# ov2slam/ov2slam

Measured on AMD Instinct MI355X. Metric: frames/sec tracking + local-BA iters/sec, EuRoC MH_01 stereo 'accurate', 1 GPU vs CPU ref, higher is better.
Workload: dtype u8/int32 fixed point + f32 (LK), f64 (BA)

## Files before the change

### ov2slam_amd/csrc/clahe.hip

```cpp
#include "common.hpp"
#include "xcd_map.hpp"
#include <math.h>
#include <mutex>
#include <type_traits>

#pragma clang fp contract(off)

__device__ __forceinline__ int c_reflect101(int p, int len)
{
    if (len == 1) return 0;
    while (p < 0 || p >= len) p = p < 0 ? -p : 2 * len - 2 - p;
    return p;
}

struct ClaheParams {
    int w, h, stride, tiles_x, tiles_y, tw, th, clip;
    float lut_scale, inv_tw, inv_th;
    long long src_item_stride, dst_item_stride;
    int dst_stride;
    int border;
    int batch, gx_lut;
    int ysplit;
    int nstrips, nlut;
    long long l1_delta;
    int l1_pitch, l1_w, l1_h;
};

__device__ __forceinline__ void clahe_wave_sync()
{
    __builtin_amdgcn_fence(__ATOMIC_RELEASE, "wavefront");
    __builtin_amdgcn_wave_barrier();
    __builtin_amdgcn_fence(__ATOMIC_ACQUIRE, "wavefront");
}

#define CH_WAVE_DW 256
#define CH_CSTRIDE 264
#define CH_NCOPY 4
#define CH_MULTI_DW (CH_NCOPY * CH_CSTRIDE)
typedef uint32_t c_u32x4 __attribute__((ext_vector_type(4)));

template <int CTRL>
__device__ __forceinline__ int c_dpp0(int v) { return __builtin_amdgcn_update_dpp(0, v, CTRL, 0xF, 0xF, true); }

template <bool SRC_ALIGNED, class StoreLut>
__device__ __forceinline__ void clahe_lut_tiles(const ClaheParams &P, const uint8_t *img, uint32_t *hw, int lane, int t, int t_end, int tstride,
                                                StoreLut store_lut, int ncopy = 1)
{
    const int ntiles = t_end;
    const int sub = lane >> 4, l16 = lane & 15;
    uint32_t *hist = hw + ((lane ^ (lane >> 4)) & (ncopy - 1)) * CH_CSTRIDE;
    const bool fast_geom = P.tw <= 61 && P.th <= 64;
    const uint8_t *img_end = img + (long long)(P.h - 1) * P.stride + P.w;
    const bool same_phase = SRC_ALIGNED || (P.stride & 3) == 0;

    auto tile_fast = [&](int t) { const int xb = (t % P.tiles_x) * P.tw; return fast_geom && 2 * xb + P.tw <= 2 * P.w - 1; };
    const uint32_t lane_off = (uint32_t)(sub * P.stride + 4 * l16);
    auto tile_load = [&](int t, uint32_t (&vv)[16], uint32_t &phs) {
        const int ty = t / P.tiles_x, tx = t - ty * P.tiles_x;
        const int x_begin = tx * P.tw;
        if (SRC_ALIGNED && (ty * P.th + 64 <= P.h) && (long long)P.h * P.stride < (1ll << 31)) {
            const uint32_t ph = (uint32_t)(x_begin & 3);
            phs = ph * 0x55555555u;
            const uint8_t *tp = img + (long long)(ty * P.th) * P.stride + (x_begin & ~3);
            uint32_t off = (4 * l16 < P.tw + (int)ph && (x_begin & ~3) + 4 * l16 < P.w) ? lane_off : (uint32_t)(sub * P.stride);
#pragma unroll
            for (int i = 0; i < 16; i++) {
                vv[i] = *(const uint32_t *)(tp + off);
                off += 4u * (uint32_t)P.stride;
            }
            return;
        }
        const int ybase = ty * P.th + sub;
        phs = 0;
#pragma unroll
        for (int i = 0; i < 16; i++) {
            int y = ybase + 4 * i;
            y = y >= P.h ? 2 * P.h - 2 - y : y;
            y = y < 0 ? 0 : y;
            uint32_t v = 0;
            if (SRC_ALIGNED) {
                const uint32_t ph = (uint32_t)(x_begin & 3);
                phs |= ph << (2 * i);
                if (4 * i + sub < P.th && 4 * l16 < P.tw + (int)ph && (x_begin & ~3) + 4 * l16 < P.w) v = *(const uint32_t *)(img + y * P.stride + (x_begin & ~3) + 4 * l16);
            } else {
                const uint8_t *rp = img + (long long)y * P.stride + x_begin;
                const uint32_t ph = (uint32_t)((size_t)rp & 3);
                phs |= ph << (2 * i);
                const uint8_t *ap = rp - ph + 4 * l16;
                if (4 * i + sub < P.th && 4 * l16 < P.tw + (int)ph && x_begin - (int)ph + 4 * l16 < P.w) {
                    if (ap + 4 <= img_end) v = *(const uint32_t *)ap;
                    else for (int k = 0; k < 4; k++) if (ap + k < img_end) v |= (uint32_t)ap[k] << (8 * k);
                }
            }
            vv[i] = v;
        }
    };

    uint32_t cur[16], cur_ph = 0;
    auto histogram = [&](int th) {
        const int ty = th / P.tiles_x, tx = th - ty * P.tiles_x;
        const int x_begin = tx * P.tw;
        if (ncopy == 1) ((c_u32x4 *)hw)[lane] = (c_u32x4)(0u);
        else for (int q = lane; q < CH_MULTI_DW / 4; q += 64) ((c_u32x4 *)hw)[q] = (c_u32x4)(0u);
        clahe_wave_sync();
        if (tile_fast(th)) {
            const int dbl_lo = 2 * P.w - 2 - (x_begin + P.tw);
            auto wgt = [&](int p) { const int c = x_begin + p; return ((unsigned)p < (unsigned)P.tw && c < P.w) ? ((c > dbl_lo && c <= P.w - 2) ? 2u : 1u) : 0u; };
            const int p_same = 4 * l16 - (int)(cur_ph & 3);
            uint32_t w0 = wgt(p_same), w1 = wgt(p_same + 1), w2 = wgt(p_same + 2), w3 = wgt(p_same + 3);
            bool mine = p_same < P.tw;
#pragma unroll
            for (int i = 0; i < 16; i++) {
                if (!same_phase) {
                    const int p0 = 4 * l16 - (int)((cur_ph >> (2 * i)) & 3);
                    w0 = wgt(p0); w1 = wgt(p0 + 1); w2 = wgt(p0 + 2); w3 = wgt(p0 + 3);
                    mine = p0 < P.tw;
                }
                if (mine && 4 * i + sub < P.th) {
                    const uint32_t v = cur[i];
                    atomicAdd(&hist[v & 0xFF], w0);
                    atomicAdd(&hist[(v >> 8) & 0xFF], w1);
                    atomicAdd(&hist[(v >> 16) & 0xFF], w2);
                    atomicAdd(&hist[v >> 24], w3);
                }
            }
        } else {
            for (int ly = sub; ly < P.th; ly += 4) {
                const uint8_t *row = img + (long long)c_reflect101(ty * P.th + ly, P.h) * P.stride;
                for (int lx = l16; lx < P.tw; lx += 16) atomicAdd(&hist[row[c_reflect101(x_begin + lx, P.w)]], 1u);
            }
        }
    };
    if (t < ntiles) {
        if (tile_fast(t)) tile_load(t, cur, cur_ph);
        histogram(t);
        if (t + tstride < ntiles && tile_fast(t + tstride)) tile_load(t + tstride, cur, cur_ph);
    }
#pragma nounroll
    for (; t < ntiles; t += tstride) {
        clahe_wave_sync();
        int hv[4];
        {
            c_u32x4 q = *(const c_u32x4 *)(hw + 4 * lane);
            for (int c = 1; c < ncopy; c++) q += *(const c_u32x4 *)(hw + c * CH_CSTRIDE + 4 * lane);
            hv[0] = (int)q.x; hv[1] = (int)q.y; hv[2] = (int)q.z; hv[3] = (int)q.w;
        }
        clahe_wave_sync();
        const int tn = t + tstride;
        if (tn < ntiles) {
            histogram(tn);
            if (tn + tstride < ntiles && tile_fast(tn + tstride)) tile_load(tn + tstride, cur, cur_ph);
        }
        if (P.clip > 0) {
            int over = 0;
#pragma unroll
            for (int k = 0; k < 4; k++) { over += max(hv[k] - P.clip, 0); hv[k] = min(hv[k], P.clip); }
            over += c_dpp0<0xB1>(over); over += c_dpp0<0x4E>(over); over += c_dpp0<0x124>(over); over += c_dpp0<0x128>(over);
            const int clipped = __builtin_amdgcn_readlane(over, 0) + __builtin_amdgcn_readlane(over, 16) +
                                __builtin_amdgcn_readlane(over, 32) + __builtin_amdgcn_readlane(over, 48);
            const int batch = clipped >> 8, residual = clipped & 255;
            int step = residual ? (int)(256.0f / (float)residual) : 1;
            int q = (int)((float)(4 * lane) / (float)step), r = 4 * lane - q * step;
#pragma unroll
            for (int k = 0; k < 4; k++) {
                hv[k] += batch + ((residual != 0 && r == 0 && q < residual) ? 1 : 0);
                r++;
                if (r == step) { r = 0; q++; }
            }
        }
        hv[1] += hv[0]; hv[2] += hv[1]; hv[3] += hv[2];
        int v = hv[3];
        v += c_dpp0<0x111>(v); v += c_dpp0<0x112>(v); v += c_dpp0<0x114>(v); v += c_dpp0<0x118>(v);
        const int r0 = __builtin_amdgcn_readlane(v, 15), r1 = __builtin_amdgcn_readlane(v, 31), r2 = __builtin_amdgcn_readlane(v, 47);
        const int rowoff = sub == 0 ? 0 : (sub == 1 ? r0 : (sub == 2 ? r0 + r1 : r0 + r1 + r2));
        const int base = v + rowoff - hv[3];
        uint32_t packed = 0;
#pragma unroll
        for (int k = 0; k < 4; k++) {
            int r = __float2int_rn((float)(hv[k] + base) * P.lut_scale);
            r = r < 0 ? 0 : (r > 255 ? 255 : r);
            packed |= (uint32_t)r << (8 * k);
        }
        store_lut(t, packed);
    }
}

template <bool SRC_ALIGNED>
__global__ __launch_bounds__(256, 4) void k_clahe_lut(ClaheParams P, const uint8_t *__restrict__ src, uint8_t *__restrict__ lut)
{
    __shared__ __attribute__((aligned(16))) uint32_t hist_all[4][CH_MULTI_DW];
    const int wave = __builtin_amdgcn_readfirstlane(threadIdx.x >> 6), lane = threadIdx.x & 63;
    const int ntiles = P.tiles_x * P.tiles_y;
    int b, bx;
    ov2_xcd_map(blockIdx.x, P.gx_lut, P.batch, &b, &bx);
    uint8_t *lb = lut + (long long)b * ntiles * 256 + 4 * lane;
    clahe_lut_tiles<SRC_ALIGNED>(P, src + (long long)b * P.src_item_stride, hist_all[wave], lane, bx * 4 + wave, ntiles, 4 * P.gx_lut,
                                 [&](int t, uint32_t packed) { *(uint32_t *)(lb + (long long)t * 256) = packed; }, CH_NCOPY);
}

#define CLAHE_MAX_CELLS 48
#define CA_UNROLL 6
typedef float c_f32x2 __attribute__((ext_vector_type(2)));

__device__ __forceinline__ float c_ub(uint32_t q, int k) { return (float)((q >> (8 * k)) & 0xFFu); }

template <bool SRC_ALIGNED>
__global__ __launch_bounds__(512) void k_clahe_apply(ClaheParams P, const uint8_t *__restrict__ src, const uint8_t *__restrict__ lut,
                                                     uint8_t *__restrict__ dst)
{
    extern __shared__ __align__(16) unsigned char clahe_smem[];
    const int ncx = P.tiles_x + 1;
    uint32_t *lut4 = (uint32_t *)clahe_smem;
    int cy, b;
    ov2_xcd_map(blockIdx.x, (P.tiles_y + 1) * P.ysplit, P.batch, &b, &cy);
    const int part = cy % P.ysplit;
    cy /= P.ysplit;
    const int tid = threadIdx.x, nthr = blockDim.x;
    const int ty1 = max(cy - 1, 0), ty2 = min(cy, P.tiles_y - 1);
    const uint8_t *L = lut + (long long)b * P.tiles_x * P.tiles_y * 256;
    for (int e = tid; e < ncx * 64; e += nthr) {
        const int cx = e >> 6, v4 = (e & 63) * 4;
        const int tx1 = max(cx - 1, 0), tx2 = min(cx, P.tiles_x - 1);
        const uint32_t a = *(const uint32_t *)(L + (ty1 * P.tiles_x + tx1) * 256 + v4), bb = *(const uint32_t *)(L + (ty1 * P.tiles_x + tx2) * 256 + v4);
        const uint32_t c = *(const uint32_t *)(L + (ty2 * P.tiles_x + tx1) * 256 + v4), d = *(const uint32_t *)(L + (ty2 * P.tiles_x + tx2) * 256 + v4);
        const uint32_t ab01 = __builtin_amdgcn_perm(bb, a, 0x05010400u), ab23 = __builtin_amdgcn_perm(bb, a, 0x07030602u);
        const uint32_t cd01 = __builtin_amdgcn_perm(d, c, 0x05010400u), cd23 = __builtin_amdgcn_perm(d, c, 0x07030602u);
        c_u32x4 o;
        o.x = __builtin_amdgcn_perm(cd01, ab01, 0x05040100u); o.y = __builtin_amdgcn_perm(cd01, ab01, 0x07060302u);
        o.z = __builtin_amdgcn_perm(cd23, ab23, 0x05040100u); o.w = __builtin_amdgcn_perm(cd23, ab23, 0x07060302u);
        *(c_u32x4 *)(lut4 + (cx << 8) + v4) = o;
    }
    __syncthreads();
    int y0 = max(0, (int)floorf(((float)cy - 0.5f) * (float)P.th) - 1), y1 = min(P.h, (int)ceilf(((float)cy + 0.5f) * (float)P.th) + 2);
    while (y0 < y1 && (int)floorf((float)y0 * P.inv_th - 0.5f) + 1 != cy) y0++;
    while (y1 > y0 && (int)floorf((float)(y1 - 1) * P.inv_th - 0.5f) + 1 != cy) y1--;
    if (P.ysplit > 1) {
        const int chunk = (y1 - y0 + P.ysplit - 1) / P.ysplit;
        y0 = min(y1, y0 + part * chunk);
        y1 = min(y1, y0 + chunk);
    }
    const uint8_t *simg = src + (long long)b * P.src_item_stride;
    uint8_t *dimg = dst + (long long)b * P.dst_item_stride;
    const bool dst_aligned = ((P.dst_stride | (int)(size_t)dimg) & 3) == 0;
    constexpr bool src_aligned = SRC_ALIGNED;
    const uint8_t *simg_end = simg + (long long)(P.h - 1) * P.stride + P.w;
    const int ndw = (P.w + 3) >> 2;
    for (int dwi = tid; dwi < ndw; dwi += nthr) {
        const int xb = 4 * dwi;
        float xa[4], xa1[4];
        const uint32_t *lutc[4];
#pragma unroll
        for (int k = 0; k < 4; k++) {
            const int x = min(xb + k, P.w - 1);
            const float txf = (float)x * P.inv_tw - 0.5f;
            const int fx = (int)floorf(txf);
            xa[k] = txf - (float)fx; xa1[k] = 1.0f - xa[k];
            lutc[k] = lut4 + ((fx + 1) << 8);
        }
        const c_f32x2 XA01 = {xa[0], xa[1]}, XA23 = {xa[2], xa[3]}, XB01 = {xa1[0], xa1[1]}, XB23 = {xa1[2], xa1[3]};
        const bool full = dst_aligned && xb + 3 < P.w;
        auto load_rows = [&](int yb, uint32_t (&inr)[CA_UNROLL]) {
#pragma unroll
            for (int u = 0; u < CA_UNROLL; u++) {
                const int y = min(yb + u, y1 - 1);
                const uint8_t *sp = simg + (long long)y * P.stride + xb;
                uint32_t in = 0;
                if (src_aligned) in = *(const uint32_t *)sp;
                else {
                    const uint32_t ph = (uint32_t)((size_t)sp & 3);
                    const uint8_t *ap = sp - ph;
                    if (xb + 3 < P.w && ap + 8 <= simg_end) {
                        const uint32_t lo = *(const uint32_t *)ap, hi = *(const uint32_t *)(ap + 4);
                        in = __builtin_amdgcn_alignbyte(hi, lo, ph);
                    } else for (int k = 0; k < 4; k++) if (xb + k < P.w) in |= (uint32_t)sp[k] << (8 * k);
                }
                inr[u] = in;
            }
        };
        uint32_t inr[CA_UNROLL], nxt[CA_UNROLL];
        if (y0 < y1) load_rows(y0, inr);
        for (int yb = y0; yb < y1; yb += CA_UNROLL) {
            load_rows(yb + CA_UNROLL, nxt);
#pragma unroll
            for (int u = 0; u < CA_UNROLL; u++) {
                const int y = yb + u;
                if (y >= y1) break;
                const float tyf = (float)y * P.inv_th - 0.5f;
                const float ya = tyf - (float)(cy - 1), ya1 = 1.0f - ya;
                const c_f32x2 YA = {ya, ya}, YB = {ya1, ya1};
                uint8_t *drow = dimg + y * P.dst_stride;
                const uint32_t in = inr[u];
                const uint32_t q0 = lutc[0][in & 0xFF], q1 = lutc[1][(in >> 8) & 0xFF], q2 = lutc[2][(in >> 16) & 0xFF], q3 = lutc[3][in >> 24];
                const c_f32x2 A11 = {c_ub(q0, 0), c_ub(q1, 0)}, A12 = {c_ub(q0, 1), c_ub(q1, 1)}, A21 = {c_ub(q0, 2), c_ub(q1, 2)}, A22 = {c_ub(q0, 3), c_ub(q1, 3)};
                const c_f32x2 B11 = {c_ub(q2, 0), c_ub(q3, 0)}, B12 = {c_ub(q2, 1), c_ub(q3, 1)}, B21 = {c_ub(q2, 2), c_ub(q3, 2)}, B22 = {c_ub(q2, 3), c_ub(q3, 3)};
                const c_f32x2 r01 = (A11 * XB01 + A12 * XA01) * YB + (A21 * XB01 + A22 * XA01) * YA;
                const c_f32x2 r23 = (B11 * XB23 + B12 * XA23) * YB + (B21 * XB23 + B22 * XA23) * YA;
                uint32_t out = __builtin_amdgcn_cvt_pk_u8_f32(rintf(r01.x), 0, 0u);
                out = __builtin_amdgcn_cvt_pk_u8_f32(rintf(r01.y), 1, out);
                out = __builtin_amdgcn_cvt_pk_u8_f32(rintf(r23.x), 2, out);
                out = __builtin_amdgcn_cvt_pk_u8_f32(rintf(r23.y), 3, out);
                if (full) *(uint32_t *)(drow + xb) = out;
                else for (int k = 0; k < 4; k++) if (xb + k < P.w) drow[xb + k] = (uint8_t)(out >> (8 * k));
            }
#pragma unroll
            for (int u = 0; u < CA_UNROLL; u++) inr[u] = nxt[u];
        }
    }
    if (P.border > 0) {
        __threadfence_block();
        __syncthreads();
        const int win = P.border, pbl = (win + 3) & ~3, wend = (P.w + win + 3) & ~3, rbeg = P.w & ~3;
        const int ndw_lr = pbl / 4 + ((wend - rbeg) >> 2), ndw_row = (pbl + wend) >> 2;
        auto put = [&](int yt, int ysrc, int c0) {
            const uint8_t *srow = dimg + ysrc * P.dst_stride;
            uint32_t v;
            if (c0 >= 0 && c0 + 3 < P.w) v = *(const uint32_t *)(srow + c0);
            else {
                v = 0;
#pragma unroll
                for (int k = 0; k < 4; k++) {
                    int c = c0 + k;
                    c = c < -win ? -win : (c > P.w + win - 1 ? P.w + win - 1 : c);
                    v |= (uint32_t)srow[c_reflect101(c, P.w)] << (8 * k);
                }
            }
            *(uint32_t *)(dimg + yt * P.dst_stride + c0) = v;
        };
        for (int row = tid >> 3; row < y1 - y0; row += nthr >> 3)
            for (int d = tid & 7; d < ndw_lr; d += 8)
                put(y0 + row, y0 + row, d < pbl / 4 ? 4 * d - pbl : rbeg + 4 * (d - pbl / 4));
        for (int k = max(1, y0); k <= min(win, y1 - 1); k++)
            for (int d = tid; d < ndw_row; d += nthr) put(-k, k, 4 * d - pbl);
        for (int k = max(1, P.h - y1); k <= min(win, P.h - 1 - y0); k++)
            for (int d = tid; d < ndw_row; d += nthr) put(P.h - 1 + k, P.h - 1 - k, 4 * d - pbl);
    }
}

__device__ __forceinline__ uint32_t c_wave_shr1(uint32_t v) { return (uint32_t)__builtin_amdgcn_update_dpp(0, (int)v, 0x138, 0xF, 0xF, true); }
__device__ __forceinline__ uint32_t c_wave_shl1(uint32_t v) { return (uint32_t)__builtin_amdgcn_update_dpp(0, (int)v, 0x130, 0xF, 0xF, true); }

#define CS_UNROLL 6
#define CS_MAX_STRIPS 8
#define CS_LUT_PRIO 3
enum { CS_MID = 0, CS_EDGE = 1, CS_ANY = 2 };
template <int E> using cs_tag = std::integral_constant<int, E>;
template <bool UNAL, bool FUSED>
__global__ __launch_bounds__(64 * (CS_MAX_STRIPS + 2), 6) void k_clahe_apply_pyr(ClaheParams P, const uint8_t *__restrict__ src, const uint8_t *__restrict__ lut,
                                                                                uint8_t *__restrict__ dst)
{
    extern __shared__ __align__(16) unsigned char clahe_smem[];
    uint32_t *lut4 = (uint32_t *)clahe_smem;
    uint8_t *ring = clahe_smem + (size_t)(P.tiles_x + 1) * 1024;
    const int b = blockIdx.x, s = __builtin_amdgcn_readfirstlane(threadIdx.x >> 6);
    const int lane = threadIdx.x & 63, ndw = (P.w + 3) >> 2, wr = UNAL ? (P.w & 3) : 0;
    uint32_t *hist_w = (uint32_t *)(ring + (size_t)2 * P.tiles_x * 256) + (s < P.nstrips ? s * CH_WAVE_DW : P.nstrips * CH_WAVE_DW + (s - P.nstrips) * CH_MULTI_DW);
    const int hist_copies = s < P.nstrips ? 1 : CH_NCOPY;
    auto lut_row = [&](int ty, int tx0, int txstep) {
        uint8_t *slot = ring + (size_t)(ty & 1) * P.tiles_x * 256 - (size_t)ty * P.tiles_x * 256 + 4 * lane;
        clahe_lut_tiles<!UNAL>(P, src + (long long)b * P.src_item_stride, hist_w, lane, ty * P.tiles_x + tx0, (ty + 1) * P.tiles_x, txstep,
                               [&](int t, uint32_t packed) { *(uint32_t *)(slot + (size_t)t * 256) = packed; }, hist_copies);
    };
    typedef uint32_t cs_u32_a1 __attribute__((aligned(1)));
    const int cmin = 0, ncell = P.tiles_x + 1;
    const uint8_t *L = lut + (long long)b * P.tiles_x * P.tiles_y * 256;
    auto cell_row = [&](int y) { return (int)floorf((float)y * P.inv_th - 0.5f) + 1; };
    int cy = -1, y_switch = 0;
    auto build = [&](int cyv) {
        const int ty1 = max(cyv - 1, 0), ty2 = min(cyv, P.tiles_y - 1);
        const uint8_t *L1 = FUSED ? ring + (size_t)(ty1 & 1) * P.tiles_x * 256 : L + (size_t)ty1 * P.tiles_x * 256;
        const uint8_t *L2 = FUSED ? ring + (size_t)(ty2 & 1) * P.tiles_x * 256 : L + (size_t)ty2 * P.tiles_x * 256;
        __syncthreads();
        for (int e = threadIdx.x; e < ncell * 64; e += blockDim.x) {
            const int cx = cmin + (e >> 6), v4 = (e & 63) * 4;
            const int tx1 = max(cx - 1, 0), tx2 = min(cx, P.tiles_x - 1);
            const uint32_t a = *(const uint32_t *)(L1 + tx1 * 256 + v4), bb = *(const uint32_t *)(L1 + tx2 * 256 + v4);
            const uint32_t c = *(const uint32_t *)(L2 + tx1 * 256 + v4), dd = *(const uint32_t *)(L2 + tx2 * 256 + v4);
            const uint32_t ab01 = __builtin_amdgcn_perm(bb, a, 0x05010400u), ab23 = __builtin_amdgcn_perm(bb, a, 0x07030602u);
            const uint32_t cd01 = __builtin_amdgcn_perm(dd, c, 0x05010400u), cd23 = __builtin_amdgcn_perm(dd, c, 0x07030602u);
            c_u32x4 o;
            o.x = __builtin_amdgcn_perm(cd01, ab01, 0x05040100u); o.y = __builtin_amdgcn_perm(cd01, ab01, 0x07060302u);
            o.z = __builtin_amdgcn_perm(cd23, ab23, 0x05040100u); o.w = __builtin_amdgcn_perm(cd23, ab23, 0x07060302u);
            *(c_u32x4 *)(lut4 + ((e >> 6) << 8) + v4) = o;
        }
        __syncthreads();
    };
    if (FUSED) {
        lut_row(0, s, P.nstrips + P.nlut);
        if (s >= P.nstrips) {
            const int n_cell_rows = cell_row(P.h - 1) + 1;
            __builtin_amdgcn_s_setprio(CS_LUT_PRIO);
            for (int c = 0; c < n_cell_rows; c++) {
                build(c);
                if (c + 1 < P.tiles_y) lut_row(c + 1, s - P.nstrips, P.nlut);
            }
            return;
        }
    }
    const int core0 = s == 0 ? 0 : 63 + 62 * (s - 1);
    const int core1 = s == P.nstrips - 1 ? ndw : 63 + 62 * s;
    const int d_first = s == 0 ? 0 : core0 - 1;
    const int d_raw = d_first + lane;
    const int d = min(d_raw, ndw - 1);
    const bool core = d_raw >= core0 && d_raw < core1;
    const int xb = 4 * d;
    float xa[4], xa1[4];
    const uint32_t *lutc[4];
#pragma unroll
    for (int k = 0; k < 4; k++) {
        const float txf = (float)min(xb + k, P.w - 1) * P.inv_tw - 0.5f;
        const int fx = (int)floorf(txf);
        xa[k] = txf - (float)fx; xa1[k] = 1.0f - xa[k];
        lutc[k] = lut4 + ((fx + 1 - cmin) << 8);
    }
    const c_f32x2 XA01 = {xa[0], xa[1]}, XA23 = {xa[2], xa[3]}, XB01 = {xa1[0], xa1[1]}, XB23 = {xa1[2], xa1[3]};
    uint8_t *dimg = dst + (long long)b * P.dst_item_stride;
    uint8_t *l1 = dimg + P.l1_delta;
    const int win = P.border;
    const int l1odd = UNAL ? (P.l1_w & 1) : 0;
    const int nb0 = (win + 3) >> 2, nb1 = (win + 1) >> 1;
    const int nbr0 = nb0 + (wr ? 1 : 0), nbr1 = nb1 + l1odd;
    const bool bl0 = core && d < nb0, br0 = core && d >= ndw - nbr0;
    const bool bl1 = core && d >= 1 && d <= nb1, br1 = core && d >= ndw - nbr1;
    const bool edge_strip = s == 0 || core1 > ndw - max(nbr0, nbr1);
    const bool first_col = d_raw == 0, last_col = d_raw == ndw - 1;
    const bool dup = d_raw > ndw - 1;
    const uint32_t pad0 = 4u * nb0, pad1 = 2u * nb1;
    const uint32_t slack0 = pad0 + 4u * (uint32_t)((P.w + win + 3) >> 2), slack1 = pad1 + 2u * (uint32_t)((P.l1_w + win + 3) >> 1);
    const uint32_t o0 = dup ? slack0 : pad0 + 4u * d;
    const uint32_t o0b = bl0 ? pad0 - 4u * (d + 1) : (br0 ? pad0 + (uint32_t)(2 * P.w - 2 - xb - ((wr & 1) ? 0 : 2)) : slack0);
    const uint32_t sel_br = (wr & 1) ? 0x01020304u : 0x03040506u;
    const uint32_t sel_fix = (last_col && wr) ? (wr == 1 ? 0x01020304u : (wr == 2 ? 0x03040504u : 0x05060504u)) : 0x07060504u;
    const uint32_t sel_rt = wr == 0 ? 0x0c0c0c06u : (wr == 1 ? 0x0c0c0c00u : (wr == 2 ? 0x0c0c0c02u : 0x0c0c0c04u));
    const uint32_t o1 = core ? pad1 + 2u * d : slack1;
    const uint32_t o1b = bl1 ? pad1 - 2u * d : (br1 ? pad1 + (uint32_t)P.l1_w + 2u * (ndw - 1 - d) - (uint32_t)l1odd : slack1);
    const bool fix1 = last_col && l1odd;
    uint8_t *d0m = dimg - pad0, *d1m = l1 - pad1;
    const uint32_t xo = (d == ndw - 1 && wr) ? (uint32_t)(P.w - 4) : (uint32_t)xb;
    const uint32_t in_sh = (d == ndw - 1 && wr) ? 8u * (4u - (uint32_t)wr) : 0u;

    int y_tab = 0;
    float wya = 0.f, wyb = 0.f;
    auto ytab = [&](int y) {
        y_tab = y;
        const float tyf = (float)(y + lane) * P.inv_th - 0.5f;
        wya = tyf - (float)(cy - 1); wyb = 1.0f - wya;
    };
    auto stage = [&](int y) {
        cy = cell_row(y);
        int yn = max(y + 1, (int)(((float)cy + 0.5f) * (float)P.th) - 2);
        while (yn < P.h && cell_row(yn) == cy) yn++;
        y_switch = yn;
        ytab(y);
        build(cy);
    };
    uint8_t *dbase = min(d0m - (long long)win * P.dst_stride, d1m - (long long)win * P.l1_pitch) - 256;
    const __amdgpu_buffer_rsrc_t rs_dst = __builtin_amdgcn_make_buffer_rsrc(dbase, 0, 0x7fffffff, 0x00020000);
    const uint8_t *sbase = src + (long long)b * P.src_item_stride;
    const __amdgpu_buffer_rsrc_t rs_src = __builtin_amdgcn_make_buffer_rsrc((void *)sbase, 0, 0x7fffffff, 0x00020000);
    const int so_d0 = (int)(d0m - dbase), so_d1 = (int)(d1m - dbase);
    const bool mid_strip = !edge_strip && d_first > 0 && d_first + 63 < ndw - 1;
    auto cs_edge = [&](auto edge_c) { return decltype(edge_c)::value == CS_EDGE || (decltype(edge_c)::value == CS_ANY && edge_strip); };
    auto put0 = [&](int so, uint32_t v, uint32_t bv, auto edge_c) {
        __builtin_amdgcn_raw_buffer_store_b32(v, rs_dst, (int)o0, so, 0);
        if (cs_edge(edge_c)) __builtin_amdgcn_raw_buffer_store_b32(bv, rs_dst, (int)o0b, so, 0);
    };
    auto put1 = [&](int so, uint32_t v, uint32_t bv, auto edge_c) {
        __builtin_amdgcn_raw_buffer_store_b16((unsigned short)v, rs_dst, (int)o1, so, 0);
        if (cs_edge(edge_c)) __builtin_amdgcn_raw_buffer_store_b16((unsigned short)bv, rs_dst, (int)o1b, so, 0);
    };
    typedef unsigned short cu16x2 __attribute__((ext_vector_type(2)));
    int r1 = so_d1;
    auto emit = [&](int Y, uint32_t c0, uint32_t c1, uint32_t c2, uint32_t c3, uint32_t c4, auto mirror_c, auto edge_c) {
        constexpr bool MIRROR = decltype(mirror_c)::value;
        const cu16x2 s0 = __builtin_bit_cast(cu16x2, c0), s1 = __builtin_bit_cast(cu16x2, c1), s2 = __builtin_bit_cast(cu16x2, c2),
                     s3 = __builtin_bit_cast(cu16x2, c3), s4 = __builtin_bit_cast(cu16x2, c4);
        const cu16x2 v = (s2 * (unsigned short)6 + (s1 + s3) * (unsigned short)4 + s0 + s4 + (unsigned short)128) >> (unsigned short)8;
        uint32_t o = __builtin_amdgcn_perm(0u, __builtin_bit_cast(uint32_t, v), 0x0c0c0200u);
        uint32_t bv = 0;
        if (cs_edge(edge_c)) {
            bv = __builtin_amdgcn_perm(c_wave_shr1(o), o, 0x0c0c0500u);
            if (UNAL && fix1) o = bv;
        }
        put1(r1, o, bv, edge_c);
        r1 += P.l1_pitch;
        if (MIRROR) {
            if (Y >= 1 && Y <= win) put1(so_d1 - Y * P.l1_pitch, o, bv, edge_c);
            if (Y >= P.l1_h - 1 - win && Y <= P.l1_h - 2) put1(so_d1 + (2 * (P.l1_h - 1) - Y) * P.l1_pitch, o, bv, edge_c);
        }
    };

    uint32_t hA = 0, hB = 0, hC = 0, hD = 0, hE = 0;
    const uint8_t *srow = src + (long long)b * P.src_item_stride;
    int r0 = so_d0;
    uint32_t inr[CS_UNROLL], nxt[CS_UNROLL];
#pragma unroll
    for (int u = 0; u < CS_UNROLL; u++) inr[u] = *(const cs_u32_a1 *)(srow + (long long)min(u, P.h - 1) * P.stride + xo) >> (UNAL ? in_sh : 0u);
    srow += (long long)CS_UNROLL * P.stride;
    auto do_row = [&](int y, uint32_t in, auto mirror_c, auto edge_c) {
        constexpr bool MIRROR = decltype(mirror_c)::value;
        constexpr int EDGE = decltype(edge_c)::value;
        const float ya = __builtin_bit_cast(float, __builtin_amdgcn_readlane(__builtin_bit_cast(int, wya), y - y_tab));
        const float ya1 = __builtin_bit_cast(float, __builtin_amdgcn_readlane(__builtin_bit_cast(int, wyb), y - y_tab));
        const c_f32x2 YA = {ya, ya}, YB = {ya1, ya1};
        const uint32_t q0 = lutc[0][in & 0xFF], q1 = lutc[1][(in >> 8) & 0xFF], q2 = lutc[2][(in >> 16) & 0xFF], q3 = lutc[3][in >> 24];
        const c_f32x2 A11 = {c_ub(q0, 0), c_ub(q1, 0)}, A12 = {c_ub(q0, 1), c_ub(q1, 1)}, A21 = {c_ub(q0, 2), c_ub(q1, 2)}, A22 = {c_ub(q0, 3), c_ub(q1, 3)};
        const c_f32x2 B11 = {c_ub(q2, 0), c_ub(q3, 0)}, B12 = {c_ub(q2, 1), c_ub(q3, 1)}, B21 = {c_ub(q2, 2), c_ub(q3, 2)}, B22 = {c_ub(q2, 3), c_ub(q3, 3)};
        const c_f32x2 r01 = (A11 * XB01 + A12 * XA01) * YB + (A21 * XB01 + A22 * XA01) * YA;
        const c_f32x2 r23 = (B11 * XB23 + B12 * XA23) * YB + (B21 * XB23 + B22 * XA23) * YA;
        const c_f32x2 MAGIC = {12582912.0f, 12582912.0f};
        const c_f32x2 m01 = r01 + MAGIC, m23 = r23 + MAGIC;
        const uint32_t u0 = __builtin_bit_cast(uint32_t, (float)m01.x), u1 = __builtin_bit_cast(uint32_t, (float)m01.y);
        const uint32_t u2 = __builtin_bit_cast(uint32_t, (float)m23.x), u3 = __builtin_bit_cast(uint32_t, (float)m23.y);
        uint32_t out = __builtin_amdgcn_perm(__builtin_amdgcn_perm(u3, u2, 0x0c0c0400u), __builtin_amdgcn_perm(u1, u0, 0x0c0c0400u), 0x05040100u);
        uint32_t lf = c_wave_shr1(out), rt = c_wave_shl1(out);
        uint32_t bv = 0;
        if (EDGE != CS_MID) {
            if (first_col) lf = __builtin_amdgcn_perm(out, out, 0x01020000u);
            if (cs_edge(edge_c)) {
                if (UNAL) out = __builtin_amdgcn_perm(out, lf, sel_fix);
            }
            if (UNAL) { if (last_col) rt = __builtin_amdgcn_perm(out, lf, sel_rt); }
            else if (last_col) rt = out >> 16;
            if (cs_edge(edge_c))
                bv = bl0 ? __builtin_amdgcn_perm(out, rt, 0x05060700u) : __builtin_amdgcn_perm(out, lf, sel_br);
        }
        put0(r0, out, bv, edge_c);
        r0 += P.dst_stride;
        if (MIRROR) {
            if (y >= 1 && y <= win) put0(so_d0 - y * P.dst_stride, out, bv, edge_c);
            if (y >= P.h - 1 - win && y <= P.h - 2) put0(so_d0 + (2 * (P.h - 1) - y) * P.dst_stride, out, bv, edge_c);
        }
        const uint32_t l0 = __builtin_amdgcn_alignbyte(out, lf, 2);
        const uint32_t h0 = __builtin_amdgcn_udot4(l0, 0x04060401u, __builtin_amdgcn_udot4(out, 0x00010000u, 0u, false), false);
        const uint32_t h1 = __builtin_amdgcn_udot4(out, 0x04060401u, __builtin_amdgcn_udot4(rt, 0x00000001u, 0u, false), false);
        hA = hB; hB = hC; hC = hD; hD = hE; hE = h0 | (h1 << 16);
    };
    const int fast_end = min(min(P.h - win - CS_UNROLL, 2 * (P.l1_h - 1 - win) - CS_UNROLL + 4), P.h - CS_UNROLL + 1);
    for (int yb = 0; yb < P.h; yb += CS_UNROLL) {
        if (yb + 2 * CS_UNROLL <= P.h) {
#pragma unroll
            for (int u = 0; u < CS_UNROLL; u++) { nxt[u] = (uint32_t)__builtin_amdgcn_raw_buffer_load_b32(rs_src, (int)xo, (int)(srow - sbase), 0) >> (UNAL ? in_sh : 0u); srow += P.stride; }
        } else {
#pragma unroll
            for (int u = 0; u < CS_UNROLL; u++)
                nxt[u] = *(const cs_u32_a1 *)(src + (long long)b * P.src_item_stride + (long long)min(yb + CS_UNROLL + u, P.h - 1) * P.stride + xo) >> (UNAL ? in_sh : 0u);
        }
        if (yb == y_switch) stage(yb);
        const bool fast = yb > 2 * win + 2 && yb < fast_end && y_switch >= yb + CS_UNROLL;
        if (fast) {
            if (yb + CS_UNROLL > y_tab + 64) ytab(yb);
            auto group = [&](auto edge_c) {
                asm volatile("; strip kind %6" : "+v"(inr[0]), "+v"(inr[1]), "+v"(inr[2]), "+v"(inr[3]), "+v"(inr[4]), "+v"(inr[5]) : "i"(decltype(edge_c)::value));
#pragma unroll
                for (int u = 0; u < CS_UNROLL; u++) {
                    do_row(yb + u, inr[u], std::false_type(), edge_c);
                    if ((u & 1) == 0) emit((yb + u - 2) >> 1, hA, hB, hC, hD, hE, std::false_type(), edge_c);
                }
            };
            if (mid_strip) group(cs_tag<CS_MID>());
            else if (edge_strip) group(cs_tag<CS_EDGE>());
            else group(cs_tag<CS_ANY>());
        } else {
#pragma nounroll
            for (int u = 0; u < CS_UNROLL; u++) {
                const int y = yb + u;
                if (y >= P.h) break;
                if (y == y_switch) stage(y);
                if (y >= y_tab + 64) ytab(y);
                do_row(y, inr[0], std::true_type(), cs_tag<CS_ANY>());
                if (!(y & 1)) {
                    if (y == 2) emit(0, hE, hD, hC, hD, hE, std::true_type(), cs_tag<CS_ANY>());
                    else if (y > 2) emit((y - 2) >> 1, hA, hB, hC, hD, hE, std::true_type(), cs_tag<CS_ANY>());
                }
#pragma unroll
                for (int k = 0; k + 1 < CS_UNROLL; k++) inr[k] = inr[k + 1];
            }
        }
#pragma unroll
        for (int u = 0; u < CS_UNROLL; u++) inr[u] = nxt[u];
    }
    if (P.h & 1) emit((P.h - 1) >> 1, hC, hD, hE, hD, hC, std::true_type(), cs_tag<CS_ANY>());
    else emit((P.h - 2) >> 1, hB, hC, hD, hE, hD, std::true_type(), cs_tag<CS_ANY>());
}

int ov2_launch_clahe(ov2_ctx *ctx, const uint8_t *src_d, int w, int h, int stride, size_t src_batch_stride, int batch,
                     double clip_limit, int tiles_x, int tiles_y, uint8_t *dst_d, int dst_stride, size_t dst_batch_stride,
                     uint8_t *lut_d, int border, const PyrDesc *pyr, int *level1_done)
{
    if (level1_done) *level1_done = 0;
    OV2_REQUIRE(tiles_x + 1 <= CLAHE_MAX_CELLS && (size_t)(tiles_x + 1) * 1024 <= 160 * 1024, OV2_EUNSUPPORTED,
                "CLAHE: too many tile columns / too wide an image for the LDS tables");
    static std::once_flag attr_once;
    static hipError_t attr_err = hipSuccess;
    std::call_once(attr_once, [] {
        attr_err = hipFuncSetAttribute((const void *)k_clahe_apply<true>, hipFuncAttributeMaxDynamicSharedMemorySize, 160 * 1024);
        if (attr_err == hipSuccess)
            attr_err = hipFuncSetAttribute((const void *)k_clahe_apply<false>, hipFuncAttributeMaxDynamicSharedMemorySize, 160 * 1024);
    });
    OV2_HIP_CHECK(attr_err);
    ClaheParams P;
    P.border = border;
    P.nstrips = 0; P.nlut = 0; P.l1_delta = 0; P.l1_pitch = P.l1_w = P.l1_h = 0;
    int ew = w, eh = h;
    if (!(w % tiles_x == 0 && h % tiles_y == 0)) { ew = w + (tiles_x - w % tiles_x); eh = h + (tiles_y - h % tiles_y); }
    P.w = w; P.h = h; P.stride = stride; P.tiles_x = tiles_x; P.tiles_y = tiles_y;
    P.tw = ew / tiles_x; P.th = eh / tiles_y;
    const int total = P.tw * P.th;
    P.lut_scale = (float)(256 - 1) / (float)total;
    P.clip = 0;
    if (clip_limit > 0.0) { P.clip = (int)(clip_limit * total / 256); if (P.clip < 1) P.clip = 1; }
    P.inv_tw = 1.0f / (float)P.tw; P.inv_th = 1.0f / (float)P.th;
    P.src_item_stride = (long long)src_batch_stride; P.dst_item_stride = (long long)dst_batch_stride; P.dst_stride = dst_stride;
    const int tiles_per_wave = (long long)batch * tiles_x * tiles_y >= 32768 ? 5 : 1;
    const bool src_al = ((stride | (int)(size_t)src_d | (int)src_batch_stride) & 3) == 0;
    P.ysplit = (long long)batch * (tiles_y + 1) >= 256 ? 1 : (P.th >= 48 ? 6 : (P.th >= 16 ? 3 : 1));
    P.batch = batch; P.gx_lut = (tiles_x * tiles_y + 4 * tiles_per_wave - 1) / (4 * tiles_per_wave);
    bool lut_launched = false;
    auto launch_lut = [&] {
        if (!lut_launched) hipLaunchKernelGGL(src_al ? k_clahe_lut<true> : k_clahe_lut<false>, dim3(P.gx_lut * batch), dim3(256), 0, ctx->stream, P, src_d, lut_d);
        lut_launched = true;
    };
    if (pyr && pyr->n_levels >= 2 && border == pyr->win && w >= 64 && h >= 8 && 2 * ((border + 3) / 4) + 1 <= (w + 3) / 4 &&
        (((size_t)dst_d | (size_t)dst_stride | dst_batch_stride) & 3) == 0 && (pyr->lv[1].img_pitch & 1) == 0) {
        const int ndw = (w + 3) / 4, nstrips = ndw <= 64 ? 1 : 2 + (ndw - 126 + 61) / 62;
        const bool want = ctx->clahe_strips >= 0 ? ctx->clahe_strips >= 1 : (long long)batch * nstrips >= 1024;
        if (want && nstrips <= CS_MAX_STRIPS && tiles_x + 1 <= 40) {
            static std::once_flag strip_once;
            static hipError_t strip_err = hipSuccess;
            std::call_once(strip_once, [] {
                const void *fn[4] = {(const void *)k_clahe_apply_pyr<false, false>, (const void *)k_clahe_apply_pyr<true, false>,
                                     (const void *)k_clahe_apply_pyr<false, true>, (const void *)k_clahe_apply_pyr<true, true>};
                for (int i = 0; i < 4 && strip_err == hipSuccess; i++) strip_err = hipFuncSetAttribute(fn[i], hipFuncAttributeMaxDynamicSharedMemorySize, 72 * 1024);
            });
            OV2_HIP_CHECK(strip_err);
            P.nstrips = nstrips;
            P.l1_delta = pyr->lv[1].img_roi - pyr->lv[0].img_roi; P.l1_pitch = pyr->lv[1].img_pitch; P.l1_w = pyr->lv[1].w; P.l1_h = pyr->lv[1].h;
            const bool unal = (w & 3) != 0 || (pyr->lv[1].w & 1) != 0;
            const int nlut = tiles_x <= 16 ? 1 : std::max(1, std::min((tiles_x + 7) / 8, CS_MAX_STRIPS + 2 - nstrips));
            const bool fused = (ctx->clahe_strips == 2 || (ctx->clahe_strips < 0 && tiles_x <= 16 * nlut)) && (unal || src_al);
            if (fused) {
                P.nlut = nlut;
                const size_t lds = (size_t)(tiles_x + 1) * 1024 + (size_t)2 * tiles_x * 256 + ((size_t)nstrips * CH_WAVE_DW + (size_t)P.nlut * CH_MULTI_DW) * 4;
                hipLaunchKernelGGL((unal ? k_clahe_apply_pyr<true, true> : k_clahe_apply_pyr<false, true>), dim3(batch), dim3(64 * (nstrips + P.nlut)), lds, ctx->stream, P, src_d, lut_d, dst_d);
            } else {
                launch_lut();
                hipLaunchKernelGGL((unal ? k_clahe_apply_pyr<true, false> : k_clahe_apply_pyr<false, false>), dim3(batch), dim3(64 * nstrips), (size_t)(tiles_x + 1) * 1024, ctx->stream, P, src_d, lut_d, dst_d);
            }
            OV2_HIP_CHECK(hipGetLastError());
            if (level1_done) *level1_done = 1;
            return OV2_OK;
        }
    }
    launch_lut();
    const size_t apply_lds = (size_t)(tiles_x + 1) * 1024;
    const int ndw = (w + 3) / 4, passes = (ndw + 511) / 512;
    const int apply_threads = (((ndw + passes - 1) / passes) + 63) / 64 * 64;
    hipLaunchKernelGGL(src_al ? k_clahe_apply<true> : k_clahe_apply<false>, dim3((tiles_y + 1) * P.ysplit * batch), dim3(apply_threads), apply_lds, ctx->stream, P, src_d, lut_d, dst_d);
    OV2_HIP_CHECK(hipGetLastError());
    return OV2_OK;
}

extern "C" {

int ov2_clahe_d(ov2_ctx *ctx, const uint8_t *src_d, int w, int h, int stride, size_t src_batch_stride, int batch,
                double clip_limit, int tiles_x, int tiles_y, uint8_t *dst_d, int dst_stride, size_t dst_batch_stride)
{
    OV2_REQUIRE(ctx && src_d && dst_d, OV2_EINVAL, "NULL argument");
    OV2_REQUIRE(w > 0 && h > 0 && stride >= w && dst_stride >= w && batch >= 1 && tiles_x > 0 && tiles_y > 0, OV2_EINVAL, "bad geometry");
    OV2_REQUIRE(tiles_x <= w && tiles_y <= h, OV2_EINVAL, "more tiles than pixels");
    OV2_HIP_CHECK(hipSetDevice(ctx->device));
    const size_t lut_bytes = (size_t)batch * tiles_x * tiles_y * 256;
    const int rc = ctx->reserve_device(lut_bytes);
    if (rc != OV2_OK) return rc;
    return ov2_launch_clahe(ctx, src_d, w, h, stride, src_batch_stride, batch, clip_limit, tiles_x, tiles_y, dst_d, dst_stride,
                            dst_batch_stride, (uint8_t *)ctx->d_scratch, 0, nullptr, nullptr);
}

int ov2_pyr_build_clahe_d(ov2_ctx *ctx, ov2_pyr *p, const uint8_t *img_d, int stride, size_t img_batch_stride,
                          double clip_limit, int tiles_x, int tiles_y)
{
    OV2_REQUIRE(ctx && p && img_d, OV2_EINVAL, "NULL argument");
    OV2_REQUIRE(stride >= p->w && tiles_x > 0 && tiles_y > 0 && tiles_x <= p->w && tiles_y <= p->h, OV2_EINVAL, "bad geometry");
    OV2_REQUIRE(p->d.batch == 1 || img_batch_stride >= (size_t)stride * (size_t)p->h, OV2_EINVAL, "img_batch_stride too small");
    OV2_HIP_CHECK(hipSetDevice(ctx->device));
    const size_t lut_bytes = (size_t)p->d.batch * tiles_x * tiles_y * 256;
    int rc = ctx->reserve_device(lut_bytes);
    if (rc != OV2_OK) return rc;
    const PyrLevelDesc &L0 = p->d.lv[0];
    int l1_done = 0;
    rc = ov2_launch_clahe(ctx, img_d, p->w, p->h, stride, img_batch_stride, p->d.batch, clip_limit, tiles_x, tiles_y,
                          p->d.base + L0.img_roi, L0.img_pitch, (size_t)p->d.item_stride, (uint8_t *)ctx->d_scratch, p->d.win,
                          &p->d, &l1_done);
    if (rc != OV2_OK) return rc;
    rc = ov2_launch_pyr_build(ctx, p, nullptr, 0, 0, l1_done);
    if (rc != OV2_OK) return rc;
    return ov2_pyr_mark_ready(ctx, p);
}

int ov2_pyr_build_clahe_h(ov2_ctx *ctx, ov2_pyr *p, const uint8_t *img_h, int stride, double clip_limit, int tiles_x, int tiles_y)
{
    OV2_REQUIRE(ctx && p && img_h, OV2_EINVAL, "NULL argument");
    OV2_REQUIRE(p->d.batch == 1, OV2_EINVAL, "host-buffer entry point takes batch=1 pyramids");
    OV2_REQUIRE(stride >= p->w && tiles_x > 0 && tiles_y > 0 && tiles_x <= p->w && tiles_y <= p->h, OV2_EINVAL, "bad geometry");
    OV2_HIP_CHECK(hipSetDevice(ctx->device));
    const size_t pitch = ((size_t)p->w + 15) & ~(size_t)15;
    const size_t img = (pitch * p->h + 255) & ~(size_t)255, lut_bytes = (size_t)tiles_x * tiles_y * 256;
    int rc = ctx->reserve_device(img + lut_bytes);
    if (rc != OV2_OK) return rc;
    uint8_t *ds = (uint8_t *)ctx->d_scratch;
    rc = ctx->upload_image(ds, pitch, img_h, (size_t)stride, (size_t)p->w, (size_t)p->h);
    if (rc != OV2_OK) return rc;
    const PyrLevelDesc &L0 = p->d.lv[0];
    int l1_done = 0;
    rc = ov2_launch_clahe(ctx, ds, p->w, p->h, (int)pitch, 0, 1, clip_limit, tiles_x, tiles_y, p->d.base + L0.img_roi, L0.img_pitch,
                          (size_t)p->d.item_stride, ds + img, p->d.win, &p->d, &l1_done);
    if (rc != OV2_OK) return rc;
    rc = ov2_launch_pyr_build(ctx, p, nullptr, 0, 0, l1_done);
    if (rc != OV2_OK) return rc;
    return ov2_pyr_mark_ready(ctx, p);
}

int ov2_pyr_build_clahe_hb(ov2_ctx *ctx, ov2_pyr *p, int n_items, const uint8_t *const *img_h, int stride, double clip_limit, int tiles_x, int tiles_y)
{
    OV2_REQUIRE(ctx && p && img_h, OV2_EINVAL, "NULL argument");
    OV2_REQUIRE(p->parent == nullptr, OV2_EINVAL, "an item view is read-only");
    OV2_REQUIRE(n_items >= 1 && n_items <= p->d.batch, OV2_EINVAL, "n_items out of range");
    const bool use_clahe = clip_limit >= 0.0;
    OV2_REQUIRE(stride >= p->w && (!use_clahe || (tiles_x > 0 && tiles_y > 0 && tiles_x <= p->w && tiles_y <= p->h)), OV2_EINVAL, "bad geometry");
    for (int b = 0; b < n_items; b++) OV2_REQUIRE(img_h[b] != nullptr, OV2_EINVAL, "NULL image");
    OV2_HIP_CHECK(hipSetDevice(ctx->device));
    const size_t pitch = ((size_t)p->w + 15) & ~(size_t)15;
    const size_t img = (pitch * p->h + 255) & ~(size_t)255, lut_bytes = use_clahe ? (size_t)n_items * tiles_x * tiles_y * 256 : 0;
    int rc = ctx->reserve_device(img * (size_t)n_items + lut_bytes);
    if (rc != OV2_OK) return rc;
    uint8_t *ds = (uint8_t *)ctx->d_scratch;
    rc = ctx->upload_images(ds, pitch, img, img_h, n_items, (size_t)stride, (size_t)p->w, (size_t)p->h);
    if (rc != OV2_OK) return rc;
    ov2_pyr q = *p;
    q.d.batch = n_items;
    if (use_clahe) {
        const PyrLevelDesc &L0 = q.d.lv[0];
        int l1_done = 0;
        rc = ov2_launch_clahe(ctx, ds, p->w, p->h, (int)pitch, img, n_items, clip_limit, tiles_x, tiles_y, q.d.base + L0.img_roi, L0.img_pitch,
                              (size_t)q.d.item_stride, ds + img * (size_t)n_items, q.d.win, &q.d, &l1_done);
        if (rc != OV2_OK) return rc;
        rc = ov2_launch_pyr_build(ctx, &q, nullptr, 0, 0, l1_done);
    } else
        rc = ov2_launch_pyr_build(ctx, &q, ds, (int)pitch, img);
    if (rc != OV2_OK) return rc;
    return ov2_pyr_mark_ready(ctx, p);
}

int ov2_clahe_h(ov2_ctx *ctx, const uint8_t *src_h, int w, int h, int stride, double clip_limit, int tiles_x, int tiles_y,
                uint8_t *dst_h, int dst_stride)
{
    OV2_REQUIRE(ctx && src_h && dst_h, OV2_EINVAL, "NULL argument");
    OV2_REQUIRE(w > 0 && h > 0 && stride >= w && dst_stride >= w && tiles_x > 0 && tiles_y > 0, OV2_EINVAL, "bad geometry");
    OV2_REQUIRE(tiles_x <= w && tiles_y <= h, OV2_EINVAL, "more tiles than pixels");
    OV2_HIP_CHECK(hipSetDevice(ctx->device));
    const size_t pitch = ((size_t)w + 15) & ~(size_t)15;
    const size_t img = (pitch * h + 255) & ~(size_t)255, lut_bytes = (size_t)tiles_x * tiles_y * 256;
    int rc = ctx->reserve_device(2 * img + lut_bytes);
    if (rc != OV2_OK) return rc;
    uint8_t *ds = (uint8_t *)ctx->d_scratch;
    rc = ctx->upload_image(ds, pitch, src_h, (size_t)stride, (size_t)w, (size_t)h);
    if (rc != OV2_OK) return rc;
    const int rc2 = ov2_launch_clahe(ctx, ds, w, h, (int)pitch, 0, 1, clip_limit, tiles_x, tiles_y, ds + img, (int)pitch, 0, ds + 2 * img, 0, nullptr, nullptr);
    if (rc2 != OV2_OK) return rc2;
    rc = ctx->download_image(dst_h, (size_t)dst_stride, ds + img, pitch, (size_t)w, (size_t)h);
    if (rc != OV2_OK) return rc;
    return OV2_OK;
}

}
```

Measured before the change: 1.233 million.

## Shrink fused CLAHE LDS footprint by aliasing strip histograms and single-buffering LUT row

The fused CLAHE apply kernel now keeps one LUT row in LDS instead of a two-row ring. The interleaved cell table is updated incrementally: the previous lower row's bytes shift into the upper slot and the new row is merged in. Strip wavefront histograms are aliased onto the cell table region, which drops their separate allocation. Together these cut per-workgroup LDS so six workgroups can fit per CU at 752x480, matching the register limit. The cost is extra read-modify-write on the table entries and reliance on ordering between histogram use and table builds.

Measured after the change: 1.244 million (median of 6 runs). About the same (+0.9%).

```diff
diff --git a/ov2slam_amd/csrc/clahe.hip b/ov2slam_amd/csrc/clahe.hip
--- a/ov2slam_amd/csrc/clahe.hip
+++ b/ov2slam_amd/csrc/clahe.hip
@@ -344,19 +344,28 @@
 #define CS_LUT_PRIO 3
 enum { CS_MID = 0, CS_EDGE = 1, CS_ANY = 2 };
 template <int E> using cs_tag = std::integral_constant<int, E>;
+__host__ __device__ constexpr size_t cs_fused_table_bytes(int tiles_x, int nstrips) { return (size_t)(tiles_x + 1 > nstrips ? tiles_x + 1 : nstrips) * 1024; }
+__host__ __device__ constexpr size_t cs_fused_lds_bytes(int tiles_x, int nstrips, int nlut)
+{
+    return cs_fused_table_bytes(tiles_x, nstrips) + (size_t)tiles_x * 256 + (size_t)nlut * CH_MULTI_DW * 4;
+}
+static_assert(CH_WAVE_DW * 4 == 1024, "a strip wavefront's histogram takes the place of one cell column of the table");
+static_assert(cs_fused_lds_bytes(15, 3, 1) == 24448 && 6 * cs_fused_lds_bytes(15, 3, 1) <= 160 * 1024,
+              "752 x 480 (15 tile columns, 3 strips, 1 LUT wavefront): six work-groups per CU by LDS, as by registers");
+static_assert(cs_fused_lds_bytes(39, CS_MAX_STRIPS, (39 + 7) / 8) <= 72 * 1024, "the widest geometry the host admits (40 cell columns) fits the limit it sets");
 template <bool UNAL, bool FUSED>
 __global__ __launch_bounds__(64 * (CS_MAX_STRIPS + 2), 6) void k_clahe_apply_pyr(ClaheParams P, const uint8_t *__restrict__ src, const uint8_t *__restrict__ lut,
                                                                                 uint8_t *__restrict__ dst)
 {
     extern __shared__ __align__(16) unsigned char clahe_smem[];
     uint32_t *lut4 = (uint32_t *)clahe_smem;
-    uint8_t *ring = clahe_smem + (size_t)(P.tiles_x + 1) * 1024;
+    uint8_t *ring = clahe_smem + cs_fused_table_bytes(P.tiles_x, P.nstrips);
     const int b = blockIdx.x, s = __builtin_amdgcn_readfirstlane(threadIdx.x >> 6);
     const int lane = threadIdx.x & 63, ndw = (P.w + 3) >> 2, wr = UNAL ? (P.w & 3) : 0;
-    uint32_t *hist_w = (uint32_t *)(ring + (size_t)2 * P.tiles_x * 256) + (s < P.nstrips ? s * CH_WAVE_DW : P.nstrips * CH_WAVE_DW + (s - P.nstrips) * CH_MULTI_DW);
+    uint32_t *hist_w = s < P.nstrips ? lut4 + s * CH_WAVE_DW : (uint32_t *)(ring + (size_t)P.tiles_x * 256) + (s - P.nstrips) * CH_MULTI_DW;
     const int hist_copies = s < P.nstrips ? 1 : CH_NCOPY;
     auto lut_row = [&](int ty, int tx0, int txstep) {
-        uint8_t *slot = ring + (size_t)(ty & 1) * P.tiles_x * 256 - (size_t)ty * P.tiles_x * 256 + 4 * lane;
+        uint8_t *slot = ring - (size_t)ty * P.tiles_x * 256 + 4 * lane;
         clahe_lut_tiles<!UNAL>(P, src + (long long)b * P.src_item_stride, hist_w, lane, ty * P.tiles_x + tx0, (ty + 1) * P.tiles_x, txstep,
                                [&](int t, uint32_t packed) { *(uint32_t *)(slot + (size_t)t * 256) = packed; }, hist_copies);
     };
@@ -367,12 +376,32 @@
     int cy = -1, y_switch = 0;
     auto build = [&](int cyv) {
         const int ty1 = max(cyv - 1, 0), ty2 = min(cyv, P.tiles_y - 1);
-        const uint8_t *L1 = FUSED ? ring + (size_t)(ty1 & 1) * P.tiles_x * 256 : L + (size_t)ty1 * P.tiles_x * 256;
-        const uint8_t *L2 = FUSED ? ring + (size_t)(ty2 & 1) * P.tiles_x * 256 : L + (size_t)ty2 * P.tiles_x * 256;
+        const uint8_t *L1 = L + (size_t)ty1 * P.tiles_x * 256, *L2 = L + (size_t)ty2 * P.tiles_x * 256;
         __syncthreads();
         for (int e = threadIdx.x; e < ncell * 64; e += blockDim.x) {
             const int cx = cmin + (e >> 6), v4 = (e & 63) * 4;
             const int tx1 = max(cx - 1, 0), tx2 = min(cx, P.tiles_x - 1);
+            if (FUSED) {
+                c_u32x4 *ent = (c_u32x4 *)(lut4 + ((e >> 6) << 8) + v4), o;
+                if (cyv < P.tiles_y) {
+                    const uint32_t c = *(const uint32_t *)(ring + tx1 * 256 + v4), dd = *(const uint32_t *)(ring + tx2 * 256 + v4);
+                    const uint32_t cd01 = __builtin_amdgcn_perm(dd, c, 0x05010400u), cd23 = __builtin_amdgcn_perm(dd, c, 0x07030602u);
+                    if (cyv == 0) {
+                        o.x = __builtin_amdgcn_perm(cd01, cd01, 0x05040100u); o.y = __builtin_amdgcn_perm(cd01, cd01, 0x07060302u);
+                        o.z = __builtin_amdgcn_perm(cd23, cd23, 0x05040100u); o.w = __builtin_amdgcn_perm(cd23, cd23, 0x07060302u);
+                    } else {
+                        o = *ent;
+                        o.x = __builtin_amdgcn_perm(cd01, o.x, 0x05040302u); o.y = __builtin_amdgcn_perm(cd01, o.y, 0x07060302u);
+                        o.z = __builtin_amdgcn_perm(cd23, o.z, 0x05040302u); o.w = __builtin_amdgcn_perm(cd23, o.w, 0x07060302u);
+                    }
+                } else {
+                    o = *ent;
+                    o.x = __builtin_amdgcn_perm(o.x, o.x, 0x07060302u); o.y = __builtin_amdgcn_perm(o.y, o.y, 0x07060302u);
+                    o.z = __builtin_amdgcn_perm(o.z, o.z, 0x07060302u); o.w = __builtin_amdgcn_perm(o.w, o.w, 0x07060302u);
+                }
+                *ent = o;
+                continue;
+            }
             const uint32_t a = *(const uint32_t *)(L1 + tx1 * 256 + v4), bb = *(const uint32_t *)(L1 + tx2 * 256 + v4);
             const uint32_t c = *(const uint32_t *)(L2 + tx1 * 256 + v4), dd = *(const uint32_t *)(L2 + tx2 * 256 + v4);
             const uint32_t ab01 = __builtin_amdgcn_perm(bb, a, 0x05010400u), ab23 = __builtin_amdgcn_perm(bb, a, 0x07030602u);
@@ -640,7 +669,7 @@
             const bool fused = (ctx->clahe_strips == 2 || (ctx->clahe_strips < 0 && tiles_x <= 16 * nlut)) && (unal || src_al);
             if (fused) {
                 P.nlut = nlut;
-                const size_t lds = (size_t)(tiles_x + 1) * 1024 + (size_t)2 * tiles_x * 256 + ((size_t)nstrips * CH_WAVE_DW + (size_t)P.nlut * CH_MULTI_DW) * 4;
+                const size_t lds = cs_fused_lds_bytes(tiles_x, nstrips, P.nlut);
                 hipLaunchKernelGGL((unal ? k_clahe_apply_pyr<true, true> : k_clahe_apply_pyr<false, true>), dim3(batch), dim3(64 * (nstrips + P.nlut)), lds, ctx->stream, P, src_d, lut_d, dst_d);
             } else {
                 launch_lut();
```
